# JiehongLin/SAM-6D

Hardware: NVIDIA H100
Metric: poses/sec (higher is better)
Workload: dtype bf16

## Files before the change

include/sam6d_b200.h:

```cpp
#ifndef SAM6D_B200_H
#define SAM6D_B200_H

#ifdef __cplusplus
extern "C" {
#endif


int sam6d_fps(const float* xyz, int b, int n, int m, float* temp, int* idx, void* stream);
int sam6d_fps_single_cta(const float* xyz, int b, int n, int m, float* temp, int* idx, void* stream);

int sam6d_gather_points(const float* points, const int* idx, int b, int c, int n, int m, float* out, void* stream);

int sam6d_gather_rows(const float* src, const int* idx, int b, int n, int m, int c, long long src_bstride, float* out,
                      void* stream);
int sam6d_gather_rows_bf16_f32(const void* src, const int* idx, int b, int n, int m, int c, long long src_bstride, float* out,
                               void* stream);

int sam6d_ball_query(const float* new_xyz, const float* xyz, int b, int n, int m, float radius, int nsample, int* idx,
                     int* cnt, void* stream);
int sam6d_ball_query_pair(const float* new_xyz, const float* xyz, int b, int n, int m, float radius_a, int nsample_a,
                          float radius_b, int nsample_b, int* idx_a, int* idx_b, int* cnt_a, int* cnt_b, void* stream);

int sam6d_group_points(const float* points, const int* idx, int b, int c, int n, int np, int ns, float* out, void* stream);

// ... 151 lines not shown
                                   const float* radius, float* R_out, float* t_out, float* score_out, unsigned char* valid,
                                   int* count, void* stream);


int sam6d_pe_mlp_max(const float* pts, const int* idx, const int* cnt, int B, int N, int ns, const float* W1,
                     const float* B1, const float* W2, const float* B2, const float* W3, const float* B3, float* out,
                     int out_ld, int out_off, void* stream);
int sam6d_pe_mlp_max_tc(const float* pts, const int* idx, int B, int N, int ns, const float* W1, const float* B1,
                        const void* W2_bf16, const float* B2, const void* W3_bf16, const float* B3, void* out, int out_is_bf16,
                        int out_ld, int out_off, void* stream);
int sam6d_fine_assign(const float* A, int B, int S, int ld, float shift, const float* pts2, float* rsum, float* csum, float* cpart,
                      int* cpi, int* lab1, int* lab2, float* wts, float* pred, void* stream);
int sam6d_fine_pass_tc(const void* Fa, const void* Fb, int B, int S, float alpha, float shift, int mode, const float* row_f,
                       const float* col_f, int ld_f, const float* q4, float* out_inv, int* lab, float* wts, float* pred, void* stream);
int sam6d_fine_masked_points(const int* lab2, const float* pts2, int B, int S, int ld, float* q4, void* stream);
int sam6d_weighted_procrustes(const float* src, const float* ref, const float* wts, int B, int N, float weight_thresh,
                              float eps, float* R, float* t, void* stream);
int sam6d_pose_score(const float* pts1, const int* lab1, int B, int N, const float* R, const float* t, const float* model,
                     int nm, float dis_thres, const float* radius, float* score, float* t_scaled, void* stream);

int sam6d_bilinear_gather(const void* up, int up_is_bf16, const long long* choose, int B, int K, int G, int sub, int C, int H, int W,
                          float* out, void* stream);

int sam6d_attn_relpos(const float* qkv, long long tok_ld, int nW, int Hs, int Ws, int nH, int head_dim, const float* rel_h,
                      const float* rel_w, float scale, void* out, int out_is_bf16, long long out_ld, void* stream);

int sam6d_attn_global_tc(const void* qkv, long long ld, const void* Vt, long long vt_ld, const void* rel_blob, int B, int H, int grid,
                         float scale, void* out, int out_is_bf16, long long out_ld, void* stream);
int sam6d_attn_global_tc_ex(const void* qkv, long long ld, const void* Vt, long long vt_ld, const void* rel_blob, int B, int H, int grid,
                            int head_dim, float scale, void* out, int out_is_bf16, long long out_ld, void* stream);
// ... 76 lines not shown
```

sam6d_b200/_lib.py:

```python
import ctypes
import os
import re

import torch

_Tensor = torch.Tensor

_HERE = os.path.dirname(os.path.abspath(__file__))
HEADER = os.path.join(os.path.dirname(_HERE), "include", "sam6d_b200.h")
LIB_PATH = os.path.join(_HERE, "libsam6d_b200.so")

_CTYPES = {
    "int": ctypes.c_int,
    "long long": ctypes.c_longlong,
    "float": ctypes.c_float,
    "double": ctypes.c_double,
}


def parse_header(path: str = HEADER):
    text = open(path).read()
    text = re.sub(r"/\*.*?\*/", "", text, flags=re.S)
    protos = {}
    for m in re.finditer(r"(const char\*|int)\s+(sam6d_\w+)\s*\(([^)]*)\)\s*;", text):
# ... 26 lines not shown
        if not os.path.exists(LIB_PATH):
            raise Sam6dError(
                f"{LIB_PATH} not found: build it with `python -m sam6d_b200.build` "
                "(or __graft_entry__.build()); sam6d_b200 has no CPU or eager fallback")
        _lib = ctypes.CDLL(LIB_PATH)
        _protos = parse_header()
        for name, (ret, args) in _protos.items():
            fn = getattr(_lib, name)
            fn.restype = ret
            fn.argtypes = [t for t, _ in args]
            _fns[name] = (fn, len(args) - 1 if args and args[-1][1] == "stream" else -1)
    return _lib


_launches = 0
_MULTI = {"sam6d_fine_assign": 6, "sam6d_coarse_select": 2, "sam6d_geo_embed_tc": 2, "sam6d_render_meshes": 4, "sam6d_yolo_masks": 2,
          "sam6d_mask_rle_count": 2, "sam6d_template_score_agg": 2, "sam6d_template_score": 2,
          "sam6d_pbr_reference_crops": 2, "sam6d_track_points": 4,
          "sam6d_track_points_scene": 5, "sam6d_symmetry_agreement": 2, "sam6d_tsdf_mesh_count": 2, "sam6d_tsdf_mesh_emit": 2}
_timed = {}


def launch_count() -> int:
    return _launches


def add_launches(n: int):
    global _launches
    _launches += int(n)


# ... 43 lines not shown
```

sam6d_b200/csrc/epilogue.cuh:

```cuda
#pragma once
#include "tc.cuh"

namespace epi {

template <int ACT>
__device__ __forceinline__ float act_fn(float x) {
  if constexpr (ACT == 1) return fmaxf(x, 0.f);
  if constexpr (ACT == 2) return 0.5f * x * (1.f + erff(x * 0.70710678118654752f));
  return x;
}

template <typename T>
struct ident { using type = T; };
__device__ __forceinline__ float ld_res(const float* p) { return *p; }
__device__ __forceinline__ float ld_res(const __nv_bfloat16* p) { return __bfloat162float(*p); }
__device__ __forceinline__ float2 ld_res2(const float* p) { return *reinterpret_cast<const float2*>(p); }
__device__ __forceinline__ float2 ld_res2(const __nv_bfloat16* p) { return __bfloat1622float2(*reinterpret_cast<const __nv_bfloat162*>(p)); }
__device__ __forceinline__ void st1(float* p, float a) { *p = a; }
__device__ __forceinline__ void st1(__nv_bfloat16* p, float a) { *p = __float2bfloat16(a); }
__device__ __forceinline__ void st2(float* p, float a, float b) { *reinterpret_cast<float2*>(p) = make_float2(a, b); }
__device__ __forceinline__ void st2(__nv_bfloat16* p, float a, float b) { *reinterpret_cast<uint32_t*>(p) = tc::pack_bf16(a, b); }

template <typename OT, int ACT, bool HAS_BIAS, bool HAS_RES, typename RT = float, int N>
__device__ __forceinline__ void store_frag(const float (&d)[N / 2], int w, int lane, int row0, int M, int col0, int N_lim, float alpha,
// ... 35 lines not shown
  for (int j = 0; j < 16; ++j) {
    const int c = tc::frag_col(4 * j, lane);
    const float g0 = __ldg(bias + col0 + c), g1 = __ldg(bias + col0 + c + 1);
    const float u0 = __ldg(bias + col0 + 128 + c), u1 = __ldg(bias + col0 + 128 + c + 1);
#pragma unroll
    for (int h = 0; h < 2; ++h) {
      const int row = row0 + tc::frag_row(2 * h, w, lane);
      if (row >= M) continue;
      const float x0 = fmaf(d[4 * j + 2 * h], alpha, g0), x1 = fmaf(d[4 * j + 2 * h + 1], alpha, g1);
      const float y0 = fmaf(d[4 * (j + 16) + 2 * h], alpha, u0), y1 = fmaf(d[4 * (j + 16) + 2 * h + 1], alpha, u1);
      st2(C + (size_t)row * ldc + out_col0 + c, x0 / (1.f + __expf(-x0)) * y0, x1 / (1.f + __expf(-x1)) * y1);
    }
  }
}

#define EPI_DISPATCH(ACT_V, BIAS_P, RES_P, ...)                                              \
  do {                                                                                       \
    const int a__ = (ACT_V);                                                                 \
    const bool b__ = (BIAS_P) != nullptr, r__ = (RES_P) != nullptr;                          \
    if (a__ == 0) {                                                                          \
      if (b__) { if (r__) { __VA_ARGS__(0, true, true); } else { __VA_ARGS__(0, true, false); } } \
      else     { if (r__) { __VA_ARGS__(0, false, true); } else { __VA_ARGS__(0, false, false); } } \
    } else if (a__ == 1) {                                                                   \
      if (b__) { if (r__) { __VA_ARGS__(1, true, true); } else { __VA_ARGS__(1, true, false); } } \
      else     { if (r__) { __VA_ARGS__(1, false, true); } else { __VA_ARGS__(1, false, false); } } \
    } else {                                                                                 \
      if (b__) { if (r__) { __VA_ARGS__(2, true, true); } else { __VA_ARGS__(2, true, false); } } \
      else     { if (r__) { __VA_ARGS__(2, false, true); } else { __VA_ARGS__(2, false, false); } } \
    }                                                                                        \
  } while (0)
// ... 3 lines not shown
```

sam6d_b200/csrc/fine_tc.cu:

```cuda
#include "common.cuh"
#include "tc.cuh"

namespace {

constexpr int BM = 128, BN = 256, BK = 64, KB = 4, STAGES = 4;
constexpr int A_KB = BM * BK * 2, B_KB = BN * BK * 2;
constexpr int CONSUMERS = 256, NUM_THREADS = CONSUMERS + 128;
constexpr int SMEM_BYTES = KB * A_KB + STAGES * B_KB + 1024;
constexpr float LOG2E = 1.4426950408889634f;

struct FArgs {
  int B, S, mode, ld_f;
  float a2, s2;
  const float* row_f;
  const float* col_f;
  const float4* q4;
  float* out_inv;
  int* lab;
  float* wts; float* pred;
};

__device__ __forceinline__ float ex2(float x) {
  float y;
  asm("ex2.approx.ftz.f32 %0, %1;" : "=f"(y) : "f"(x));
// ... 136 lines not shown
        }
      }
    }
  }
}

__global__ void fine_masked_points_kernel(const int* __restrict__ lab2, const float* __restrict__ pts2, int S, int ld, float4* __restrict__ q4) {
  const int b = blockIdx.y, j = blockIdx.x * blockDim.x + threadIdx.x;
  if (j >= ld) return;
  float4 q = make_float4(0.f, 0.f, 0.f, 0.f);
  if (j >= 1 && j < S && lab2[(size_t)b * S + j] > 0) {
    const float* p = pts2 + ((size_t)b * (S - 1) + (j - 1)) * 3;
    q = make_float4(p[0], p[1], p[2], 1.f);
  }
  q4[(size_t)b * ld + j] = q;
}

}

S6_API int sam6d_fine_pass_tc(const void* Fa, const void* Fb, int B, int S, float alpha, float shift, int mode, const float* row_f,
                              const float* col_f, int ld_f, const float* q4, float* out_inv, int* lab, float* wts, float* pred,
                              void* stream) {
  S6_REQUIRE(Fa && Fb && B >= 0 && S >= 2 && mode >= 0 && mode <= 2 && ld_f >= S);
  S6_REQUIRE(((reinterpret_cast<uintptr_t>(Fa) | reinterpret_cast<uintptr_t>(Fb)) & 15) == 0 && (long long)B * S < 2000000000LL);
  if (mode == 0) S6_REQUIRE(out_inv != nullptr);
  if (mode >= 1) S6_REQUIRE(row_f && col_f && lab);
  if (mode == 2) S6_REQUIRE(q4 && wts && pred && (reinterpret_cast<uintptr_t>(q4) & 15) == 0);
  if (B == 0) return 0;
  CUtensorMap tmA, tmB;
  int rc = tc::make_map_2d(&tmA, Fa, (long long)B * S, 256, 256, 64, BM);
// ... 11 lines not shown
  } while (0)
  if (mode == 0) FINE_LAUNCH(0); else if (mode == 1) FINE_LAUNCH(1); else FINE_LAUNCH(2);
#undef FINE_LAUNCH
  S6_LAUNCH_CHECK();
  return 0;
}

S6_API int sam6d_fine_masked_points(const int* lab2, const float* pts2, int B, int S, int ld, float* q4, void* stream) {
  S6_REQUIRE(lab2 && pts2 && q4 && B >= 0 && S >= 2 && ld >= S && (reinterpret_cast<uintptr_t>(q4) & 15) == 0);
  if (B == 0) return 0;
  dim3 grid(s6_cdiv(ld, 256), B);
  fine_masked_points_kernel<<<grid, 256, 0, s6_stream(stream)>>>(lab2, pts2, S, ld, reinterpret_cast<float4*>(q4));
  S6_LAUNCH_CHECK();
  return 0;
}
```

sam6d_b200/csrc/gemm_tma.cu:

```cuda
#include "epilogue.cuh"
#include "tc.cuh"

namespace {

constexpr int BM = 128, BN = 256, BK = 64, STAGES = 4;
constexpr int A_BYTES = BM * BK * 2, B_BYTES = BN * BK * 2, STAGE_BYTES = A_BYTES + B_BYTES;
constexpr int CONSUMERS = 256, THREADS = CONSUMERS + 128;
constexpr int SMEM = STAGES * STAGE_BYTES + 1024;

struct Args {
  const float* bias; const void* R; void* C;
  int M, N, K;
  long long ldc, ldr;
  float alpha;
  int act;
  int batch;
  long long a_rpb, w_rpb;
  long long c_bs, r_bs;
  void* vt; int vt_col0, vt_S, vt_N1, vt_C;
  int vt_col1; void* c2; long long ldc2;
};

template <typename OT, int ACT, bool HAS_BIAS, bool HAS_RES, bool VT = false>
__global__ void __launch_bounds__(THREADS, 1) gemm_tma_kernel(const __grid_constant__ CUtensorMap tmA,
// ... 79 lines not shown
          const int row = row0 + tc::frag_row(2 * h, w, lane);
          if (row >= g.M) continue;
          const int cloud = row / g.vt_S, tok = row - cloud * g.vt_S;
#pragma unroll
          for (int e = 0; e < 2; ++e) {
            const int col = n0 + tc::frag_col(4 * j + e, lane);
            float x = acc[4 * j + 2 * h + e] * g.alpha;
            if constexpr (HAS_BIAS) x += __ldg(g.bias + col);
            reinterpret_cast<__nv_bfloat16*>(g.vt)[((size_t)cloud * g.vt_C + (col - g.vt_col0)) * g.vt_N1 + tok] =
                __float2bfloat16(epi::act_fn<ACT>(x));
          }
        }
      }
    } else if constexpr (ACT == 3) {
      epi::store_frag_swiglu(acc, w, lane, row0, g.M, n0, n0 / 2, g.alpha, g.bias, Cb, g.ldc);
    } else {
      epi::store_frag<OT, ACT, HAS_BIAS, HAS_RES, OT, BN>(acc, w, lane, row0, g.M, n0, g.N, g.alpha, g.bias, Rb, g.ldr, Cb, g.ldc);
    }
  }
}

int launch_gemm_tma(const void* A, const void* W, const float* bias, const void* R, void* C, int c_dtype, int M, int N, int K,
                    long long lda, long long ldw, long long ldc, long long ldr, int batch, long long a_rpb, long long w_rpb,
                    long long c_bs, long long r_bs, float alpha, int act, void* stream, void* vt = nullptr, int vt_col0 = 0, int vt_S = 1,
                    int vt_N1 = 0, int vt_col1 = -1, void* c2 = nullptr, long long ldc2 = 0) {
  S6_REQUIRE(A && W && C && M >= 0 && N > 0 && K > 0 && (K % 8) == 0 && (lda % 8) == 0 && (ldw % 8) == 0 && act >= 0 && act <= 3);
  S6_REQUIRE((reinterpret_cast<uintptr_t>(A) & 15) == 0 && (reinterpret_cast<uintptr_t>(W) & 15) == 0 && batch >= 0);
  S6_REQUIRE(a_rpb * (long long)batch < 2000000000LL && w_rpb * (long long)batch < 2000000000LL);
  if (M == 0 || batch == 0) return 0;
  CUtensorMap tmA, tmW;
  const long long a_rows = batch > 1 ? a_rpb * (batch - 1) + M : M, w_rows = batch > 1 ? w_rpb * (batch - 1) + N : N;
  int rc = tc::make_map_2d(&tmA, A, a_rows, K, lda, 64, BM);
  if (rc) return rc;
  rc = tc::make_map_2d(&tmW, W, w_rows, K, ldw, 64, BN);
  if (rc) return rc;
  const long long ntiles = (long long)s6_cdiv(M, BM) * s6_cdiv(N, BN) * batch;
  int grid;
  S6_CHECK(s6_persistent_grid(ntiles, 1, &grid));
  if (vt_col1 < 0) vt_col1 = N;
  Args g{bias, R, C, M, N, K, ldc, ldr, alpha, act, batch, a_rpb, w_rpb, c_bs, r_bs, vt, vt_col0, vt_S, vt_N1, vt_col1 - vt_col0,
         vt_col1, c2, ldc2};
// ... 11 lines not shown
  if (vt) {
    S6_REQUIRE(c_dtype == 1 && bias && !R && act == 0 && batch == 1 && vt_col0 > 0 && vt_col0 < N && (vt_col0 % 32) == 0 && vt_S > 0 &&
               vt_N1 >= vt_S);
    S6_REQUIRE(vt_col1 > vt_col0 && vt_col1 <= N && (vt_col1 % 32) == 0 &&
               (vt_col1 == N || (c2 && (ldc2 % 8) == 0 && ldc2 >= N - vt_col1 && (reinterpret_cast<uintptr_t>(c2) & 15) == 0)));
    LAUNCH_ONE(__nv_bfloat16, 0, true, false, true);
    S6_LAUNCH_CHECK();
    return 0;
  }
  if (act == 3) {
    S6_REQUIRE(c_dtype == 1 && bias && !R && (N % BN) == 0 && (ldc % 2) == 0 && ldc >= N / 2);
    LAUNCH_ONE(__nv_bfloat16, 3, true, false, false);
    S6_LAUNCH_CHECK();
    return 0;
  }
  EPI_DISPATCH(act, bias, R, LAUNCH_TMA);
#undef LAUNCH_TMA
#undef LAUNCH_ONE
  S6_LAUNCH_CHECK();
  return 0;
}

}

S6_API int sam6d_gemm_tma(const void* A, const void* W, const float* bias, const void* R, void* C, int c_dtype, int M, int N, int K,
                          long long lda, long long ldw, long long ldc, long long ldr, float alpha, int act, void* stream) {
  return launch_gemm_tma(A, W, bias, R, C, c_dtype, M, N, K, lda, ldw, ldc, ldr, 1, 0, 0, 0, 0, alpha, act, stream);
}

S6_API int sam6d_gemm_tma_batched(const void* A, const void* W, const float* bias, const void* R, void* C, int c_dtype, int M, int N,
// ... 20 lines not shown
```

sam6d_b200/ops.py:

```python
import math
from typing import Optional, Tuple

import numpy as np
import torch

from . import _lib

Tensor = torch.Tensor


def _check(t: Tensor, dtype, name: str, ndim: Optional[int] = None):
    if not isinstance(t, torch.Tensor):
        raise RuntimeError(f"{name} must be a torch.Tensor")
    if not t.is_cuda:
        raise RuntimeError(f"{name} must be a CUDA tensor (CPU not supported)")
    if t.dtype != dtype:
        raise RuntimeError(f"{name} must be {dtype}, got {t.dtype}")
    if not t.is_contiguous():
        raise RuntimeError(f"{name} must be contiguous")
    if ndim is not None and t.dim() != ndim:
        raise RuntimeError(f"{name} must have {ndim} dims, got {t.dim()}")


def _rows(t: Tensor) -> Tuple[int, int, int]:
# ... 113 lines not shown
    _lib.call("sam6d_gemm_bf16", A, _DT[A.dtype], W, _DT[W.dtype], bias, residual, out, _DT[out.dtype], *_gemm_dims(A, W, residual, out),
              alpha, relu)
    return out


def gemm_tma(A: Tensor, W: Tensor, bias: Optional[Tensor] = None, residual: Optional[Tensor] = None, out: Optional[Tensor] = None,
             act: int = 0, alpha: float = 1.0, out_dtype=torch.float32) -> Tensor:
    _check(A, torch.bfloat16, "A", 2)
    _check(W, torch.bfloat16, "W", 2)
    M, K = A.shape
    N = W.shape[0]
    if W.shape[1] != K:
        raise RuntimeError("gemm: inner dimensions differ")
    Nout = N // 2 if act == ACT_SWIGLU else N
    if out is None:
        out = torch.empty(M, Nout, dtype=torch.bfloat16 if act == ACT_SWIGLU else out_dtype, device=A.device)
    if residual is not None:
        _check(residual, out.dtype, "residual", 2)
    _lib.call("sam6d_gemm_tma", A, W, bias, residual, out, _DT[out.dtype], M, N, K, K, K, Nout, N, alpha, int(act))
    return out


ACT_GELU = 2
ACT_SWIGLU = 3


def pack_swiglu_rows(t: Tensor, block: int = 128) -> Tensor:
    H = t.shape[0] // 2
    if t.shape[0] != 2 * H or H % block:
        raise ValueError(f"SwiGLU w12 needs 2H rows with H % {block} == 0, got {t.shape[0]}")
    rest = t.shape[1:]
    return t.reshape(2, H // block, block, *rest).transpose(0, 1).reshape(2 * H, *rest).contiguous()


_VT_CACHE = {}


def _vt_buffer(rows: int, n1: int, device, slot: int) -> Tensor:
    key = (rows, n1, str(device), slot, torch.cuda.current_stream(device).cuda_stream)
# ... 557 lines not shown
    wts = torch.empty(B, S - 1, dtype=torch.float32, device=dev)
    pred = torch.empty(B, S - 1, 3, dtype=torch.float32, device=dev)
    _lib.call("sam6d_fine_assign", A, B, S, int(ld), shift, pts2, rsum, csum, cpart, cpi, lab1, lab2, wts, pred)
    return lab1, lab2, wts, pred


def fine_assign_tc(f1n: Tensor, f2n: Tensor, pts2: Tensor, alpha: float):
    _check(f1n, torch.bfloat16, "f1n", 3)
    _check(f2n, torch.bfloat16, "f2n", 3)
    _check(pts2, torch.float32, "pts2", 3)
    B, S, C = f1n.shape
    if C != 256 or f2n.shape != f1n.shape or pts2.shape[1] != S - 1:
        raise RuntimeError("fine_assign_tc: (B,S,256) tokens and (B,S-1,3) points expected")
    dev = f1n.device
    ld = (S + 3) // 4 * 4
    rinv = torch.empty(B, ld, dtype=torch.float32, device=dev)
    cinv = torch.empty(B, ld, dtype=torch.float32, device=dev)
    q4 = torch.empty(B, ld, 4, dtype=torch.float32, device=dev)
    lab1 = torch.zeros(B, S, dtype=torch.int32, device=dev)
    lab2 = torch.zeros(B, S, dtype=torch.int32, device=dev)
    wts = torch.empty(B, S - 1, dtype=torch.float32, device=dev)
    pred = torch.empty(B, S - 1, 3, dtype=torch.float32, device=dev)
    _lib.call("sam6d_fine_pass_tc", f1n, f2n, B, S, alpha, alpha, 0, None, None, ld, None, rinv, None, None, None)
    _lib.call("sam6d_fine_pass_tc", f2n, f1n, B, S, alpha, alpha, 0, None, None, ld, None, cinv, None, None, None)
    _lib.call("sam6d_fine_pass_tc", f2n, f1n, B, S, alpha, alpha, 1, cinv, rinv, ld, None, None, lab2, None, None)
    _lib.call("sam6d_fine_masked_points", lab2, pts2, B, S, ld, q4)
    _lib.call("sam6d_fine_pass_tc", f1n, f2n, B, S, alpha, alpha, 2, rinv, cinv, ld, q4, None, lab1, wts, pred)
    return lab1, lab2, wts, pred


def weighted_procrustes(src: Tensor, ref: Tensor, wts: Tensor, weight_thresh: float = 0.0, eps: float = 1e-5):
    _check(src, torch.float32, "src", 3)
    _check(ref, torch.float32, "ref", 3)
    _check(wts, torch.float32, "weights", 2)
    B, N, _ = src.shape
    R = torch.empty(B, 3, 3, dtype=torch.float32, device=src.device)
    t = torch.empty(B, 3, dtype=torch.float32, device=src.device)
    _lib.call("sam6d_weighted_procrustes", src, ref, wts, B, N, weight_thresh, eps, R, t)
    return R, t


def pose_score(pts1: Tensor, lab1: Tensor, R: Tensor, t: Tensor, model: Tensor, radius: Tensor, dis_thres: float = 0.15):
# ... 348 lines not shown
```

sam6d_b200/pem.py:

```python
import math
from types import SimpleNamespace
from typing import Dict, Optional

import torch
import torch.nn as nn

from . import ops
from .layers import _W, _f32, _gemm, _Packed, _param_key, PRECISIONS

NUM_HEADS = 4

RPE_TC = True
PADDED_BIAS = True
GEO_LUT_INV_H = 8.0
GEO_LUT_D_MAX = 32.0


def _cfg(cfg, **defaults):
    if isinstance(cfg, dict):
        cfg = SimpleNamespace(**cfg)
    for k, v in defaults.items():
        if not hasattr(cfg, k):
            setattr(cfg, k, v)
    return cfg
# ... 614 lines not shown
    def forward(self, p1, f1, geo1, fps_idx1, p2, f2, geo2, fps_idx2, radius, end_points):
        if self.training:
            raise NotImplementedError("sam6d_b200 implements the inference path (model.eval())")
        p1, p2 = p1.contiguous(), p2.contiguous()
        p1_ = ops.rigid_warp(p1, end_points['init_R'].contiguous(), end_points['init_t'].contiguous())
        if p1.shape == p2.shape:
            e = self._embed(_pair(f1, f2), torch.cat([p1_, p2], dim=0))
            f1, f2 = e[:p1.shape[0]], e[p1.shape[0]:]
        else:
            f1 = self._embed(f1.contiguous(), p1_)
            f2 = self._embed(f2.contiguous(), p2)
        for blk in self.transformers:
            f1, f2 = blk(f1, geo1, fps_idx1, f2, geo2, fps_idx2)
        B, S, H = f1.shape
        w = self._weights()
        if f1.shape == f2.shape:
            o = _gemm(self.precision, _pair(f1, f2).reshape(2 * B * S, H), w["w_out"], w["b_out"]).view(2 * B, S, -1)
            o1, o2 = o[:B], o[B:]
        else:
            o1 = _gemm(self.precision, f1.reshape(B * S, H), w["w_out"], w["b_out"]).view(B, S, -1)
            o2 = _gemm(self.precision, f2.reshape(B * S, H), w["w_out"], w["b_out"]).view(B, S, -1)
        model = ops.scale_by_radius(end_points['model'].contiguous(), radius.contiguous())
        if (self.precision == "bf16" and self.cfg.sim_type == 'cosine' and self.cfg.normalize_feat and H == 256
                and o1.shape[-1] == 256 and not self.return_feat):
            f1n, f2n = ops.l2norm_rows_bf16(o1.contiguous()), ops.l2norm_rows_bf16(o2.contiguous())
            lab1, _, wts, pred = ops.fine_assign_tc(f1n, f2n, p2, 1.0 / self.cfg.temp)
            pred_R, pred_t = ops.weighted_procrustes(pred, p1, wts, 0.0, 1e-5)
            score, t_scaled = ops.pose_score(p1, lab1, pred_R, pred_t, model.contiguous(), radius.contiguous(), 0.15)
        else:
            if not self.cfg.normalize_feat:
                raise NotImplementedError("FinePointMatching: normalize_feat=False scores are unbounded; the fixed-shift assignment "
                                          "kernels need cosine similarities (the SAM-6D configuration)")
            atten = compute_feature_similarity(o1, o2, self.cfg.sim_type, self.cfg.temp, self.cfg.normalize_feat, self.precision)
            pred_R, _, score, t_scaled = compute_fine_Rt(atten, p1, p2, model, temp=self.cfg.temp, radius=radius.contiguous(),
                                                         check_bound=False)
        end_points['pred_R'] = pred_R
        end_points['pred_t'] = t_scaled
        end_points['pred_pose_score'] = score
        if self.return_feat:
            return end_points, o1, o2
        return end_points


DEFAULT_MODEL_CFG = dict(
# ... 145 lines not shown
```

Before: 2644.

## Fuse L2 norm into output GEMM and restructure fine assignment into three passes

Folds the per-row L2 normalisation into the output-projection GEMM epilogue (new ACT_L2NORM), which removes the separate normalisation kernels and an intermediate buffer. The fine-matching dual softmax assignment is rebuilt. The four similarity GEMM passes plus the masked-points kernel become three TMA/wgmma passes. The first pass computes row sums and column partial sums together, the second does column argmax with packed keys and merges into labels and masked points, and the third does row assignment. This cuts one full S×S tensor-core pass and several launches, at the cost of extra partial-sum and key buffers and small merge kernels.

New measurement: 2725, median of 6. +3.0%, better.

```diff
diff --git a/include/sam6d_b200.h b/include/sam6d_b200.h
--- a/include/sam6d_b200.h
+++ b/include/sam6d_b200.h
@@ -189,6 +189,14 @@
 int sam6d_fine_pass_tc(const void* Fa, const void* Fb, int B, int S, float alpha, float shift, int mode, const float* row_f,
                        const float* col_f, int ld_f, const float* q4, float* out_inv, int* lab, float* wts, float* pred, void* stream);
 int sam6d_fine_masked_points(const int* lab2, const float* pts2, int B, int S, int ld, float* q4, void* stream);
+int sam6d_fine_sums_tc(const void* F1, const void* F2, int B, int S, float alpha, float shift, int ld, float* e0r, float* e0c,
+                       float* cpart, float* rinv, float* cinv, void* stream);
+int sam6d_fine_collabel_tc(const void* F1, const void* F2, int B, int S, float alpha, float shift, int ld, const float* e0r,
+                           const float* e0c, const float* rinv, const float* cinv, const float* pts2, void* ckey, int* lab1,
+                           int* lab2, float* q4, void* stream);
+int sam6d_fine_rowassign_tc(const void* F1, const void* F2, int B, int S, float alpha, float shift, int ld, const float* e0c,
+                            const float* rinv, const float* cinv, const float* q4, int* lab1, float* wts, float* pred,
+                            void* stream);
 int sam6d_weighted_procrustes(const float* src, const float* ref, const float* wts, int B, int N, float weight_thresh,
                               float eps, float* R, float* t, void* stream);
 int sam6d_pose_score(const float* pts1, const int* lab1, int B, int N, const float* R, const float* t, const float* model,
diff --git a/sam6d_b200/_lib.py b/sam6d_b200/_lib.py
--- a/sam6d_b200/_lib.py
+++ b/sam6d_b200/_lib.py
@@ -64,7 +64,7 @@
 
 
 _launches = 0
-_MULTI = {"sam6d_fine_assign": 6, "sam6d_coarse_select": 2, "sam6d_geo_embed_tc": 2, "sam6d_render_meshes": 4, "sam6d_yolo_masks": 2,
+_MULTI = {"sam6d_fine_assign": 6, "sam6d_fine_sums_tc": 3, "sam6d_fine_collabel_tc": 2, "sam6d_coarse_select": 2, "sam6d_geo_embed_tc": 2, "sam6d_render_meshes": 4, "sam6d_yolo_masks": 2,
           "sam6d_mask_rle_count": 2, "sam6d_template_score_agg": 2, "sam6d_template_score": 2,
           "sam6d_pbr_reference_crops": 2, "sam6d_track_points": 4,
           "sam6d_track_points_scene": 5, "sam6d_symmetry_agreement": 2, "sam6d_tsdf_mesh_count": 2, "sam6d_tsdf_mesh_emit": 2}
diff --git a/sam6d_b200/csrc/epilogue.cuh b/sam6d_b200/csrc/epilogue.cuh
--- a/sam6d_b200/csrc/epilogue.cuh
+++ b/sam6d_b200/csrc/epilogue.cuh
@@ -73,6 +73,31 @@
   }
 }
 
+__device__ __forceinline__ void store_frag_l2norm(float (&d)[128], int w, int lane, int row0, int M, float alpha,
+                                                  const float* __restrict__ bias, __nv_bfloat16* __restrict__ C, long long ldc) {
+  float ss[2] = {0.f, 0.f};
+#pragma unroll
+  for (int j = 0; j < 32; ++j) {
+    const int c = tc::frag_col(4 * j, lane);
+    const float b0 = __ldg(bias + c), b1 = __ldg(bias + c + 1);
+#pragma unroll
+    for (int h = 0; h < 2; ++h) {
+      const float x0 = fmaf(d[4 * j + 2 * h], alpha, b0), x1 = fmaf(d[4 * j + 2 * h + 1], alpha, b1);
+      d[4 * j + 2 * h] = x0; d[4 * j + 2 * h + 1] = x1;
+      ss[h] += x0 * x0 + x1 * x1;
+    }
+  }
+#pragma unroll
+  for (int h = 0; h < 2; ++h) {
+    const float n = fmaxf(sqrtf(tc::quad_sum(ss[h])), 1e-12f);
+    const int row = row0 + tc::frag_row(2 * h, w, lane);
+    if (row >= M) continue;
+#pragma unroll
+    for (int j = 0; j < 32; ++j)
+      st2(C + (size_t)row * ldc + tc::frag_col(4 * j, lane), d[4 * j + 2 * h] / n, d[4 * j + 2 * h + 1] / n);
+  }
+}
+
 #define EPI_DISPATCH(ACT_V, BIAS_P, RES_P, ...)                                              \
   do {                                                                                       \
     const int a__ = (ACT_V);                                                                 \
diff --git a/sam6d_b200/csrc/fine_tc.cu b/sam6d_b200/csrc/fine_tc.cu
--- a/sam6d_b200/csrc/fine_tc.cu
+++ b/sam6d_b200/csrc/fine_tc.cu
@@ -174,6 +174,358 @@
     q = make_float4(p[0], p[1], p[2], 1.f);
   }
   q4[(size_t)b * ld + j] = q;
+}
+
+
+__device__ __forceinline__ unsigned long long amax_key(float p, int i) {
+  return ((unsigned long long)__float_as_uint(p) << 32) | (unsigned)(~i);
+}
+__device__ __forceinline__ int amax_index(unsigned long long k) { return (int)(~(unsigned)k); }
+__device__ __forceinline__ unsigned long long kmax(unsigned long long a, unsigned long long b) { return a > b ? a : b; }
+
+__device__ __forceinline__ int red_col(int k, int lane) { return 8 * (k >> 1) + 2 * (lane & 3) + (k & 1); }
+__device__ __forceinline__ float bit_sel(unsigned m, float a, float b) {
+  return __uint_as_float((__float_as_uint(a) & m) | (__float_as_uint(b) & ~m));
+}
+__device__ __forceinline__ unsigned long long bit_sel(unsigned m, unsigned long long a, unsigned long long b) {
+  const unsigned long long m2 = ((unsigned long long)m << 32) | m;
+  return (a & m2) | (b & ~m2);
+}
+template <int H, typename T, typename Op>
+__device__ __forceinline__ void col_round(T (&v)[64], int lane, Op op) {
+  const unsigned hi = 0u - (unsigned)((lane >> (H == 32 ? 4 : H == 16 ? 3 : 2)) & 1);
+#pragma unroll
+  for (int k = 0; k < H; ++k) {
+    const T lo = v[k], up = v[k + H];
+    v[k] = op(bit_sel(hi, up, lo), __shfl_xor_sync(0xffffffffu, bit_sel(hi, lo, up), H / 2));
+  }
+}
+template <typename T, typename Op>
+__device__ __forceinline__ void warp_col_reduce(T (&v)[64], int lane, Op op) {
+  col_round<32>(v, lane, op);
+  col_round<16>(v, lane, op);
+  col_round<8>(v, lane, op);
+}
+
+struct F3Args {
+  int B, S, ld, m_tiles;
+  float a2, s2;
+  const float* e0r;
+  const float* e0c;
+  float* rinv;
+  const float* cinv;
+  const float4* q4;
+  float* cpart;
+  unsigned long long* ckey;
+  int* lab;
+  float* wts; float* pred;
+};
+
+template <int MODE>
+__global__ void __launch_bounds__(NUM_THREADS, 1) fine_pass3_kernel(const __grid_constant__ CUtensorMap tmA, const __grid_constant__ CUtensorMap tmB, F3Args g) {
+  extern __shared__ __align__(1024) uint8_t smem_raw[];
+  uint8_t* smem = reinterpret_cast<uint8_t*>((reinterpret_cast<uintptr_t>(smem_raw) + 1023) & ~(uintptr_t)1023);
+  uint8_t* a_res = smem;
+  uint8_t* ring = smem + KB * A_KB;
+  __shared__ __align__(8) uint64_t a_full, a_empty, full_bar[STAGES], empty_bar[STAGES];
+  __shared__ float sc[2][BN];
+  __shared__ __align__(16) float4 sq[2][MODE == 2 ? BN : 1];
+  __shared__ __align__(16) unsigned long long red[MODE == 2 ? 1 : CONSUMERS / 32][BN];
+
+  const int tid = threadIdx.x, warp = tid >> 5, lane = tid & 31;
+  const int S = g.S, T = S - 1;
+  const int m_tiles = g.m_tiles, n_tiles = (T + BN - 1) / BN;
+  const int items = g.B * m_tiles;
+
+  if (tid == 0) {
+    tc::mbar_init(&a_full, 1); tc::mbar_init(&a_empty, CONSUMERS / 32);
+    for (int s = 0; s < STAGES; ++s) { tc::mbar_init(&full_bar[s], 1); tc::mbar_init(&empty_bar[s], CONSUMERS / 32); }
+    tc::mbar_fence_init();
+    tc::tma_prefetch_desc(&tmA);
+    tc::tma_prefetch_desc(&tmB);
+  }
+  __syncthreads();
+
+  if (warp >= CONSUMERS / 32) {
+    tc::producer_regs();
+    if (tid == CONSUMERS) {
+      long long gk = 0;
+      int it = 0;
+      for (int item = blockIdx.x; item < items; item += gridDim.x, ++it) {
+        const int b = item / m_tiles, mt = item - b * m_tiles;
+        tc::mbar_wait(&a_empty, (uint32_t)((it & 1) ^ 1));
+        tc::mbar_arrive_expect_tx(&a_full, KB * A_KB);
+        for (int kb = 0; kb < KB; ++kb) tc::tma_load_2d(&tmA, &a_full, a_res + kb * A_KB, kb * BK, b * S + 1 + mt * BM);
+        for (int nt = 0; nt < n_tiles; ++nt)
+          for (int kb = 0; kb < KB; ++kb, ++gk) {
+            const int s = (int)(gk % STAGES);
+            tc::mbar_wait(&empty_bar[s], (uint32_t)(((gk / STAGES) & 1) ^ 1));
+            tc::mbar_arrive_expect_tx(&full_bar[s], B_KB);
+            tc::tma_load_2d(&tmB, &full_bar[s], ring + s * B_KB, kb * BK, b * S + 1 + nt * BN);
+          }
+      }
+    }
+    return;
+  }
+  tc::consumer_regs();
+  const int wg = warp >> 2, w = warp & 3;
+  const uint32_t a_addr = tc::smem_u32(a_res) + wg * (64 * 128);
+  long long gk = 0, tcount = 0;
+  int it = 0;
+  for (int item = blockIdx.x; item < items; item += gridDim.x, ++it) {
+    const int b = item / m_tiles, mt = item - b * m_tiles;
+    const size_t bo = (size_t)b * g.ld;
+    int row[2];
+    bool rv[2];
+    float rf[2] = {0.f, 0.f};
+#pragma unroll
+    for (int hr = 0; hr < 2; ++hr) {
+      row[hr] = 1 + mt * BM + wg * 64 + tc::frag_row(2 * hr, w, lane);
+      rv[hr] = row[hr] < S;
+      if (MODE != 0 && rv[hr]) rf[hr] = g.rinv[bo + row[hr]];
+    }
+    float sum[2] = {0.f, 0.f}, ws[2] = {0.f, 0.f}, px[2] = {0.f, 0.f}, py[2] = {0.f, 0.f}, pz[2] = {0.f, 0.f};
+    float bv[2] = {-INFINITY, -INFINITY};
+    int bi[2] = {0x7fffffff, 0x7fffffff};
+    if (MODE == 2) {
+      const float cf0 = g.cinv[bo];
+#pragma unroll
+      for (int hr = 0; hr < 2; ++hr)
+        if (rv[hr]) { const float e = g.e0c[bo + row[hr]]; bv[hr] = (e * rf[hr]) * (e * cf0); bi[hr] = 0; }
+    }
+    tc::mbar_wait(&a_full, (uint32_t)(it & 1));
+    for (int nt = 0; nt < n_tiles; ++nt, ++tcount) {
+      const int buf = (int)(tcount & 1);
+      {
+        const int j = 1 + nt * BN + tid;
+        if (MODE != 0) sc[buf][tid] = (j < S) ? g.cinv[bo + j] : 0.f;
+        if (MODE == 2) sq[buf][tid] = (j < S) ? g.q4[bo + j] : make_float4(0.f, 0.f, 0.f, 0.f);
+        tc::named_bar(1, CONSUMERS);
+      }
+      float acc[BN / 2];
+      int prev = -1;
+      for (int kb = 0; kb < KB; ++kb, ++gk) {
+        const int s = (int)(gk % STAGES);
+        tc::mbar_wait(&full_bar[s], (uint32_t)((gk / STAGES) & 1));
+        const uint32_t b_addr = tc::smem_u32(ring + s * B_KB);
+        tc::wg_fence();
+#pragma unroll
+        for (int k = 0; k < BK / 16; ++k)
+          tc::wgmma_bf16<BN>(acc, tc::wg_desc(a_addr + kb * A_KB + k * 32), tc::wg_desc(b_addr + k * 32), (kb | k) ? 1u : 0u);
+        tc::wg_commit();
+        if (prev >= 0) {
+          tc::wg_wait<1>();
+          if (lane == 0) tc::mbar_arrive(&empty_bar[prev]);
+        }
+        prev = s;
+      }
+      tc::wg_wait<0>();
+      if (lane == 0) tc::mbar_arrive(&empty_bar[prev]);
+      if (nt == n_tiles - 1 && lane == 0) tc::mbar_arrive(&a_empty);
+      if (MODE == 0) {
+        float cs[64];
+#pragma unroll
+        for (int e = 0; e < BN / 2; ++e) {
+          const int hr = (e >> 1) & 1, k = ((e >> 2) << 1) | (e & 1), j = 1 + nt * BN + tc::frag_col(e, lane);
+          const float ev = (j < S) ? ex2(fmaf(acc[e], g.a2, -g.s2)) : 0.f;
+          sum[hr] += ev;
+          const float c = rv[hr] ? ev : 0.f;
+          cs[k] = hr ? cs[k] + c : c;
+        }
+        warp_col_reduce(cs, lane, [](float x, float y) { return x + y; });
+        float* redf = reinterpret_cast<float*>(&red[0][0]);
+#pragma unroll
+        for (int k = 0; k < 8; ++k) redf[warp * BN + red_col(k + 8 * (lane >> 2), lane)] = cs[k];
+        tc::named_bar(1, CONSUMERS);
+        const int j = 1 + nt * BN + tid;
+        if (j < S) {
+          float t = 0.f;
+#pragma unroll
+          for (int v = 0; v < CONSUMERS / 32; ++v) t += redf[v * BN + tid];
+          g.cpart[((size_t)b * m_tiles + mt) * g.ld + j] = t;
+        }
+      } else if (MODE == 1) {
+        unsigned long long ck[64];
+#pragma unroll
+        for (int e = 0; e < BN / 2; ++e) {
+          const int hr = (e >> 1) & 1, k = ((e >> 2) << 1) | (e & 1), cl = tc::frag_col(e, lane);
+          const float ev = ex2(fmaf(acc[e], g.a2, -g.s2));
+          const unsigned long long key = rv[hr] ? amax_key((ev * rf[hr]) * (ev * sc[buf][cl]), row[hr]) : 0ull;
+          ck[k] = hr ? kmax(ck[k], key) : key;
+        }
+        warp_col_reduce(ck, lane, kmax);
+#pragma unroll
+        for (int k = 0; k < 8; ++k) red[warp][red_col(k + 8 * (lane >> 2), lane)] = ck[k];
+        tc::named_bar(1, CONSUMERS);
+        const int j = 1 + nt * BN + tid;
+        if (j < S) {
+          unsigned long long t = red[0][tid];
+#pragma unroll
+          for (int v = 1; v < CONSUMERS / 32; ++v) t = kmax(t, red[v][tid]);
+          g.ckey[((size_t)b * m_tiles + mt) * g.ld + j] = t;
+        }
+      } else {
+#pragma unroll
+        for (int e = 0; e < BN / 2; ++e) {
+          const int hr = (e >> 1) & 1, cl = tc::frag_col(e, lane), j = 1 + nt * BN + cl;
+          const float ev = (j < S) ? ex2(fmaf(acc[e], g.a2, -g.s2)) : 0.f;
+          const float p = (ev * rf[hr]) * (ev * sc[buf][cl]);
+          if (p > bv[hr]) { bv[hr] = p; bi[hr] = j; }
+          const float4 q = sq[buf][cl];
+          const float pm = p * q.w;
+          ws[hr] += pm; px[hr] = fmaf(pm, q.x, px[hr]); py[hr] = fmaf(pm, q.y, py[hr]); pz[hr] = fmaf(pm, q.z, pz[hr]);
+        }
+      }
+    }
+#pragma unroll
+    for (int hr = 0; hr < 2; ++hr) {
+      const int i = row[hr];
+      if (MODE == 0) {
+        const float t = tc::quad_sum(sum[hr]);
+        if ((lane & 3) == 0 && rv[hr]) g.rinv[bo + i] = 1.f / (g.e0c[bo + i] + t);
+      } else if (MODE == 2) {
+#pragma unroll
+        for (int o = 1; o <= 2; o <<= 1) {
+          const float ov = __shfl_xor_sync(0xffffffffu, bv[hr], o);
+          const int oi = __shfl_xor_sync(0xffffffffu, bi[hr], o);
+          if (ov > bv[hr] || (ov == bv[hr] && oi < bi[hr])) { bv[hr] = ov; bi[hr] = oi; }
+        }
+        float ww = tc::quad_sum(ws[hr]), qx = tc::quad_sum(px[hr]), qy = tc::quad_sum(py[hr]), qz = tc::quad_sum(pz[hr]);
+        if ((lane & 3) == 0 && rv[hr]) {
+          const int lb = bi[hr];
+          g.lab[(size_t)b * S + i] = lb;
+          if (lb == 0) { ww = 0.f; qx = 0.f; qy = 0.f; qz = 0.f; }
+          const size_t o = (size_t)b * (S - 1) + (i - 1);
+          const float d = ww + 1e-6f;
+          g.wts[o] = ww;
+          g.pred[o * 3 + 0] = qx / d; g.pred[o * 3 + 1] = qy / d; g.pred[o * 3 + 2] = qz / d;
+        }
+      }
+    }
+  }
+}
+
+__global__ void fine_bg_kernel(const __nv_bfloat16* __restrict__ F1, const __nv_bfloat16* __restrict__ F2, int S, int ld, float a2,
+                               float s2, float* __restrict__ e0r, float* __restrict__ e0c) {
+  const int b = blockIdx.y, lane = threadIdx.x & 31, idx = blockIdx.x * (blockDim.x >> 5) + (threadIdx.x >> 5);
+  if (idx >= S) return;
+  const bool col = blockIdx.z != 0;
+  const size_t base = (size_t)b * S * 256;
+  const uint4 x = reinterpret_cast<const uint4*>(F1 + base + (size_t)(col ? idx : 0) * 256)[lane];
+  const uint4 y = reinterpret_cast<const uint4*>(F2 + base + (size_t)(col ? 0 : idx) * 256)[lane];
+  const __nv_bfloat162* xp = reinterpret_cast<const __nv_bfloat162*>(&x);
+  const __nv_bfloat162* yp = reinterpret_cast<const __nv_bfloat162*>(&y);
+  float d = 0.f;
+#pragma unroll
+  for (int k = 0; k < 4; ++k) {
+    const float2 xf = __bfloat1622float2(xp[k]), yf = __bfloat1622float2(yp[k]);
+    d = fmaf(xf.x, yf.x, d);
+    d = fmaf(xf.y, yf.y, d);
+  }
+#pragma unroll
+  for (int o = 16; o >= 1; o >>= 1) d += __shfl_xor_sync(0xffffffffu, d, o);
+  if (lane == 0) (col ? e0c : e0r)[(size_t)b * ld + idx] = ex2(fmaf(d, a2, -s2));
+}
+
+__device__ __forceinline__ float block_sum(float v, float* sh) {
+#pragma unroll
+  for (int o = 16; o >= 1; o >>= 1) v += __shfl_xor_sync(0xffffffffu, v, o);
+  __syncthreads();
+  if ((threadIdx.x & 31) == 0) sh[threadIdx.x >> 5] = v;
+  __syncthreads();
+  float t = 0.f;
+  for (int w = 0; w < (int)(blockDim.x >> 5); ++w) t += sh[w];
+  return t;
+}
+__device__ __forceinline__ unsigned long long block_kmax(unsigned long long v, unsigned long long* sh) {
+#pragma unroll
+  for (int o = 16; o >= 1; o >>= 1) v = kmax(v, __shfl_xor_sync(0xffffffffu, v, o));
+  __syncthreads();
+  if ((threadIdx.x & 31) == 0) sh[threadIdx.x >> 5] = v;
+  __syncthreads();
+  unsigned long long t = 0;
+  for (int w = 0; w < (int)(blockDim.x >> 5); ++w) t = kmax(t, sh[w]);
+  return t;
+}
+
+__global__ void fine_sums_merge_kernel(const float* __restrict__ e0r, const float* __restrict__ e0c, const float* __restrict__ cpart,
+                                       int S, int ld, int m_tiles, float* __restrict__ rinv, float* __restrict__ cinv) {
+  __shared__ float sh[32];
+  const int b = blockIdx.y, j = blockIdx.x * blockDim.x + threadIdx.x;
+  const size_t bo = (size_t)b * ld;
+  if (j >= 1 && j < S) {
+    float t = e0r[bo + j];
+    for (int mt = 0; mt < m_tiles; ++mt) t += cpart[((size_t)b * m_tiles + mt) * ld + j];
+    cinv[bo + j] = 1.f / t;
+  }
+  if (blockIdx.x != 0) return;
+  float r = 0.f, c = 0.f;
+  for (int k = threadIdx.x; k < S; k += blockDim.x) { r += e0r[bo + k]; c += e0c[bo + k]; }
+  r = block_sum(r, sh);
+  c = block_sum(c, sh);
+  if (threadIdx.x == 0) { rinv[bo] = 1.f / r; cinv[bo] = 1.f / c; }
+}
+
+__global__ void fine_collabel_merge_kernel(const float* __restrict__ e0r, const float* __restrict__ e0c, const float* __restrict__ rinv,
+                                           const float* __restrict__ cinv, const unsigned long long* __restrict__ ckey,
+                                           const float* __restrict__ pts2, int S, int ld, int m_tiles, int* __restrict__ lab1,
+                                           int* __restrict__ lab2, float4* __restrict__ q4) {
+  __shared__ unsigned long long sh[32];
+  const int b = blockIdx.y, j = blockIdx.x * blockDim.x + threadIdx.x;
+  const size_t bo = (size_t)b * ld;
+  const float r0 = rinv[bo], c0 = cinv[bo];
+  if (j < ld) {
+    float4 q = make_float4(0.f, 0.f, 0.f, 0.f);
+    if (j >= 1 && j < S) {
+      const float e = e0r[bo + j];
+      unsigned long long t = amax_key((e * r0) * (e * cinv[bo + j]), 0);
+      for (int mt = 0; mt < m_tiles; ++mt) t = kmax(t, ckey[((size_t)b * m_tiles + mt) * ld + j]);
+      const int lb = amax_index(t);
+      lab2[(size_t)b * S + j] = lb;
+      if (lb > 0) {
+        const float* p = pts2 + ((size_t)b * (S - 1) + (j - 1)) * 3;
+        q = make_float4(p[0], p[1], p[2], 1.f);
+      }
+    }
+    q4[bo + j] = q;
+  }
+  if (blockIdx.x != 0) return;
+  unsigned long long kc = 0, kr = 0;
+  for (int k = threadIdx.x; k < S; k += blockDim.x) {
+    const float ec = e0c[bo + k], er = e0r[bo + k];
+    kc = kmax(kc, amax_key((ec * rinv[bo + k]) * (ec * c0), k));
+    kr = kmax(kr, amax_key((er * r0) * (er * cinv[bo + k]), k));
+  }
+  kc = block_kmax(kc, sh);
+  kr = block_kmax(kr, sh);
+  if (threadIdx.x == 0) { lab2[(size_t)b * S] = amax_index(kc); lab1[(size_t)b * S] = amax_index(kr); }
+}
+
+template <int MODE>
+int fine_pass3_launch(const void* F1, const void* F2, int B, int S, const F3Args& g, cudaStream_t st) {
+  CUtensorMap tmA, tmB;
+  int rc = tc::make_map_2d(&tmA, F1, (long long)B * S, 256, 256, 64, BM);
+  if (rc) return rc;
+  rc = tc::make_map_2d(&tmB, F2, (long long)B * S, 256, 256, 64, BN);
+  if (rc) return rc;
+  int grid;
+  S6_CHECK(s6_persistent_grid(B * g.m_tiles, 1, &grid));
+  S6_CHECK(cudaFuncSetAttribute(fine_pass3_kernel<MODE>, cudaFuncAttributeMaxDynamicSharedMemorySize, SMEM_BYTES));
+  fine_pass3_kernel<MODE><<<grid, NUM_THREADS, SMEM_BYTES, st>>>(tmA, tmB, g);
+  S6_LAUNCH_CHECK();
+  return 0;
+}
+
+F3Args f3_args(int B, int S, int ld, float alpha, float shift) {
+  F3Args g{};
+  g.B = B; g.S = S; g.ld = ld; g.m_tiles = s6_cdiv(S - 1, BM);
+  g.a2 = alpha * LOG2E; g.s2 = shift * LOG2E;
+  return g;
+}
+
+bool f3_tokens_ok(const void* F1, const void* F2, int B, int S, int ld) {
+  return F1 && F2 && B >= 0 && S >= 2 && ld >= S && ld % 2 == 0 && (long long)B * S < 2000000000LL &&
+         ((reinterpret_cast<uintptr_t>(F1) | reinterpret_cast<uintptr_t>(F2)) & 15) == 0;
 }
 
 }
@@ -215,3 +567,48 @@
   S6_LAUNCH_CHECK();
   return 0;
 }
+
+S6_API int sam6d_fine_sums_tc(const void* F1, const void* F2, int B, int S, float alpha, float shift, int ld, float* e0r, float* e0c,
+                              float* cpart, float* rinv, float* cinv, void* stream) {
+  S6_REQUIRE(f3_tokens_ok(F1, F2, B, S, ld) && e0r && e0c && cpart && rinv && cinv);
+  if (B == 0) return 0;
+  cudaStream_t st = s6_stream(stream);
+  F3Args g = f3_args(B, S, ld, alpha, shift);
+  fine_bg_kernel<<<dim3(s6_cdiv(S, 8), B, 2), 256, 0, st>>>(static_cast<const __nv_bfloat16*>(F1), static_cast<const __nv_bfloat16*>(F2),
+                                                             S, ld, g.a2, g.s2, e0r, e0c);
+  S6_LAUNCH_CHECK();
+  g.e0c = e0c; g.rinv = rinv; g.cpart = cpart;
+  int rc = fine_pass3_launch<0>(F1, F2, B, S, g, st);
+  if (rc) return rc;
+  fine_sums_merge_kernel<<<dim3(s6_cdiv(S, 256), B), 256, 0, st>>>(e0r, e0c, cpart, S, ld, g.m_tiles, rinv, cinv);
+  S6_LAUNCH_CHECK();
+  return 0;
+}
+
+S6_API int sam6d_fine_collabel_tc(const void* F1, const void* F2, int B, int S, float alpha, float shift, int ld, const float* e0r,
+                                  const float* e0c, const float* rinv, const float* cinv, const float* pts2, void* ckey, int* lab1,
+                                  int* lab2, float* q4, void* stream) {
+  S6_REQUIRE(f3_tokens_ok(F1, F2, B, S, ld) && e0r && e0c && rinv && cinv && pts2 && ckey && lab1 && lab2 && q4);
+  S6_REQUIRE(((reinterpret_cast<uintptr_t>(q4) | reinterpret_cast<uintptr_t>(ckey)) & 15) == 0);
+  if (B == 0) return 0;
+  cudaStream_t st = s6_stream(stream);
+  F3Args g = f3_args(B, S, ld, alpha, shift);
+  g.rinv = const_cast<float*>(rinv); g.cinv = cinv; g.ckey = static_cast<unsigned long long*>(ckey);
+  int rc = fine_pass3_launch<1>(F1, F2, B, S, g, st);
+  if (rc) return rc;
+  fine_collabel_merge_kernel<<<dim3(s6_cdiv(ld, 256), B), 256, 0, st>>>(e0r, e0c, rinv, cinv, g.ckey, pts2, S, ld, g.m_tiles, lab1,
+                                                                       lab2, reinterpret_cast<float4*>(q4));
+  S6_LAUNCH_CHECK();
+  return 0;
+}
+
+S6_API int sam6d_fine_rowassign_tc(const void* F1, const void* F2, int B, int S, float alpha, float shift, int ld, const float* e0c,
+                                   const float* rinv, const float* cinv, const float* q4, int* lab1, float* wts, float* pred,
+                                   void* stream) {
+  S6_REQUIRE(f3_tokens_ok(F1, F2, B, S, ld) && e0c && rinv && cinv && q4 && lab1 && wts && pred);
+  S6_REQUIRE((reinterpret_cast<uintptr_t>(q4) & 15) == 0);
+  if (B == 0) return 0;
+  F3Args g = f3_args(B, S, ld, alpha, shift);
+  g.e0c = e0c; g.rinv = const_cast<float*>(rinv); g.cinv = cinv; g.q4 = reinterpret_cast<const float4*>(q4); g.lab = lab1; g.wts = wts; g.pred = pred;
+  return fine_pass3_launch<2>(F1, F2, B, S, g, s6_stream(stream));
+}
diff --git a/sam6d_b200/csrc/gemm_tma.cu b/sam6d_b200/csrc/gemm_tma.cu
--- a/sam6d_b200/csrc/gemm_tma.cu
+++ b/sam6d_b200/csrc/gemm_tma.cu
@@ -117,6 +117,8 @@
       }
     } else if constexpr (ACT == 3) {
       epi::store_frag_swiglu(acc, w, lane, row0, g.M, n0, n0 / 2, g.alpha, g.bias, Cb, g.ldc);
+    } else if constexpr (ACT == 4) {
+      epi::store_frag_l2norm(acc, w, lane, row0, g.M, g.alpha, g.bias, Cb, g.ldc);
     } else {
       epi::store_frag<OT, ACT, HAS_BIAS, HAS_RES, OT, BN>(acc, w, lane, row0, g.M, n0, g.N, g.alpha, g.bias, Rb, g.ldr, Cb, g.ldc);
     }
@@ -127,7 +129,7 @@
                     long long lda, long long ldw, long long ldc, long long ldr, int batch, long long a_rpb, long long w_rpb,
                     long long c_bs, long long r_bs, float alpha, int act, void* stream, void* vt = nullptr, int vt_col0 = 0, int vt_S = 1,
                     int vt_N1 = 0, int vt_col1 = -1, void* c2 = nullptr, long long ldc2 = 0) {
-  S6_REQUIRE(A && W && C && M >= 0 && N > 0 && K > 0 && (K % 8) == 0 && (lda % 8) == 0 && (ldw % 8) == 0 && act >= 0 && act <= 3);
+  S6_REQUIRE(A && W && C && M >= 0 && N > 0 && K > 0 && (K % 8) == 0 && (lda % 8) == 0 && (ldw % 8) == 0 && act >= 0 && act <= 4);
   S6_REQUIRE((reinterpret_cast<uintptr_t>(A) & 15) == 0 && (reinterpret_cast<uintptr_t>(W) & 15) == 0 && batch >= 0);
   S6_REQUIRE(a_rpb * (long long)batch < 2000000000LL && w_rpb * (long long)batch < 2000000000LL);
   if (M == 0 || batch == 0) return 0;
@@ -169,6 +171,12 @@
     S6_LAUNCH_CHECK();
     return 0;
   }
+  if (act == 4) {
+    S6_REQUIRE(c_dtype == 1 && bias && !R && N == BN && batch == 1 && (ldc % 2) == 0 && ldc >= N);
+    LAUNCH_ONE(__nv_bfloat16, 4, true, false, false);
+    S6_LAUNCH_CHECK();
+    return 0;
+  }
   EPI_DISPATCH(act, bias, R, LAUNCH_TMA);
 #undef LAUNCH_TMA
 #undef LAUNCH_ONE
diff --git a/sam6d_b200/ops.py b/sam6d_b200/ops.py
--- a/sam6d_b200/ops.py
+++ b/sam6d_b200/ops.py
@@ -151,7 +151,7 @@
         raise RuntimeError("gemm: inner dimensions differ")
     Nout = N // 2 if act == ACT_SWIGLU else N
     if out is None:
-        out = torch.empty(M, Nout, dtype=torch.bfloat16 if act == ACT_SWIGLU else out_dtype, device=A.device)
+        out = torch.empty(M, Nout, dtype=torch.bfloat16 if act in (ACT_SWIGLU, ACT_L2NORM) else out_dtype, device=A.device)
     if residual is not None:
         _check(residual, out.dtype, "residual", 2)
     _lib.call("sam6d_gemm_tma", A, W, bias, residual, out, _DT[out.dtype], M, N, K, K, K, Nout, N, alpha, int(act))
@@ -160,6 +160,7 @@
 
 ACT_GELU = 2
 ACT_SWIGLU = 3
+ACT_L2NORM = 4
 
 
 def pack_swiglu_rows(t: Tensor, block: int = 128) -> Tensor:
@@ -747,18 +748,20 @@
         raise RuntimeError("fine_assign_tc: (B,S,256) tokens and (B,S-1,3) points expected")
     dev = f1n.device
     ld = (S + 3) // 4 * 4
-    rinv = torch.empty(B, ld, dtype=torch.float32, device=dev)
-    cinv = torch.empty(B, ld, dtype=torch.float32, device=dev)
+    m_tiles = (S - 1 + 127) // 128
+    e0 = torch.empty(2, B, ld, dtype=torch.float32, device=dev)
+    inv = torch.empty(2, B, ld, dtype=torch.float32, device=dev)
+    cpart = torch.empty(B, m_tiles, ld, dtype=torch.float32, device=dev)
+    ckey = torch.empty(B, m_tiles, ld, dtype=torch.int64, device=dev)
     q4 = torch.empty(B, ld, 4, dtype=torch.float32, device=dev)
-    lab1 = torch.zeros(B, S, dtype=torch.int32, device=dev)
-    lab2 = torch.zeros(B, S, dtype=torch.int32, device=dev)
+    lab1 = torch.empty(B, S, dtype=torch.int32, device=dev)
+    lab2 = torch.empty(B, S, dtype=torch.int32, device=dev)
     wts = torch.empty(B, S - 1, dtype=torch.float32, device=dev)
     pred = torch.empty(B, S - 1, 3, dtype=torch.float32, device=dev)
-    _lib.call("sam6d_fine_pass_tc", f1n, f2n, B, S, alpha, alpha, 0, None, None, ld, None, rinv, None, None, None)
-    _lib.call("sam6d_fine_pass_tc", f2n, f1n, B, S, alpha, alpha, 0, None, None, ld, None, cinv, None, None, None)
-    _lib.call("sam6d_fine_pass_tc", f2n, f1n, B, S, alpha, alpha, 1, cinv, rinv, ld, None, None, lab2, None, None)
-    _lib.call("sam6d_fine_masked_points", lab2, pts2, B, S, ld, q4)
-    _lib.call("sam6d_fine_pass_tc", f1n, f2n, B, S, alpha, alpha, 2, rinv, cinv, ld, q4, None, lab1, wts, pred)
+    e0r, e0c, rinv, cinv = e0[0], e0[1], inv[0], inv[1]
+    _lib.call("sam6d_fine_sums_tc", f1n, f2n, B, S, alpha, alpha, ld, e0r, e0c, cpart, rinv, cinv)
+    _lib.call("sam6d_fine_collabel_tc", f1n, f2n, B, S, alpha, alpha, ld, e0r, e0c, rinv, cinv, pts2, ckey, lab1, lab2, q4)
+    _lib.call("sam6d_fine_rowassign_tc", f1n, f2n, B, S, alpha, alpha, ld, e0c, rinv, cinv, q4, lab1, wts, pred)
     return lab1, lab2, wts, pred
 
 
diff --git a/sam6d_b200/pem.py b/sam6d_b200/pem.py
--- a/sam6d_b200/pem.py
+++ b/sam6d_b200/pem.py
@@ -652,20 +652,26 @@
             f1, f2 = blk(f1, geo1, fps_idx1, f2, geo2, fps_idx2)
         B, S, H = f1.shape
         w = self._weights()
-        if f1.shape == f2.shape:
-            o = _gemm(self.precision, _pair(f1, f2).reshape(2 * B * S, H), w["w_out"], w["b_out"]).view(2 * B, S, -1)
-            o1, o2 = o[:B], o[B:]
-        else:
-            o1 = _gemm(self.precision, f1.reshape(B * S, H), w["w_out"], w["b_out"]).view(B, S, -1)
-            o2 = _gemm(self.precision, f2.reshape(B * S, H), w["w_out"], w["b_out"]).view(B, S, -1)
         model = ops.scale_by_radius(end_points['model'].contiguous(), radius.contiguous())
         if (self.precision == "bf16" and self.cfg.sim_type == 'cosine' and self.cfg.normalize_feat and H == 256
-                and o1.shape[-1] == 256 and not self.return_feat):
-            f1n, f2n = ops.l2norm_rows_bf16(o1.contiguous()), ops.l2norm_rows_bf16(o2.contiguous())
+                and self.cfg.out_dim == 256 and not self.return_feat):
+            L2 = ops.ACT_L2NORM
+            if f1.shape == f2.shape:
+                fn = ops.gemm_tma(_pair(f1, f2).reshape(2 * B * S, H), w["w_out"].bf16, w["b_out"], act=L2).view(2 * B, S, -1)
+                f1n, f2n = fn[:B], fn[B:]
+            else:
+                f1n = ops.gemm_tma(f1.reshape(B * S, H).contiguous(), w["w_out"].bf16, w["b_out"], act=L2).view(B, S, -1)
+                f2n = ops.gemm_tma(f2.reshape(B * S, H).contiguous(), w["w_out"].bf16, w["b_out"], act=L2).view(B, S, -1)
             lab1, _, wts, pred = ops.fine_assign_tc(f1n, f2n, p2, 1.0 / self.cfg.temp)
             pred_R, pred_t = ops.weighted_procrustes(pred, p1, wts, 0.0, 1e-5)
             score, t_scaled = ops.pose_score(p1, lab1, pred_R, pred_t, model.contiguous(), radius.contiguous(), 0.15)
         else:
+            if f1.shape == f2.shape:
+                o = _gemm(self.precision, _pair(f1, f2).reshape(2 * B * S, H), w["w_out"], w["b_out"]).view(2 * B, S, -1)
+                o1, o2 = o[:B], o[B:]
+            else:
+                o1 = _gemm(self.precision, f1.reshape(B * S, H), w["w_out"], w["b_out"]).view(B, S, -1)
+                o2 = _gemm(self.precision, f2.reshape(B * S, H), w["w_out"], w["b_out"]).view(B, S, -1)
             if not self.cfg.normalize_feat:
                 raise NotImplementedError("FinePointMatching: normalize_feat=False scores are unbounded; the fixed-shift assignment "
                                           "kernels need cosine similarities (the SAM-6D configuration)")
```
